# bbuhrow/avx-ecm

Measured on AMD Instinct MI355X. Metric: stage-1 curves/sec at B1=1000000, 416-bit N, higher is better.
Workload: dtype u32 (28-bit limbs, 64-bit accumulate)

## Files before the change

### avx-ecm_amd/csrc/gecm_row.hpp

```cpp
#pragma once
#include "gecm_curve.hpp"
#include "gecm_rowk.h"

template <int NQ>
struct FeR {
    int32_t v[NQ];
};

template <int NQ>
struct RowMod {
    uint32_t n[NQ];
    uint32_t rho;
    int32_t c16;
    int32_t kb, zb;
};

__device__ __forceinline__ void row_pin(const int64_t &x)
{
    asm volatile("" ::"v"(x));
}
__device__ __forceinline__ int32_t row_c16()
{
    int32_t c;
    asm volatile("s_mov_b32 %0, 16" : "=s"(c));
    return c;
}
template <int32_t V>
__device__ __forceinline__ int32_t row_bias()
{
    int32_t c;
    asm volatile("v_mov_b32 %0, %1" : "=v"(c) : "n"(V));
    return c;
}

#define GECM_DPP_ROW_SHL1 0x101
#define GECM_DPP_ROW_SHR1 0x111
#define GECM_DPP_ROW_ROR1 0x121
#define GECM_DPP_ROW_NEWBCAST 0x150

template <int CTRL>
__device__ __forceinline__ uint32_t row_dpp(uint32_t x)
{
    return (uint32_t)__builtin_amdgcn_update_dpp(0, (int)x, CTRL, 0xF, 0xF, true);
}
template <int I>
__device__ __forceinline__ uint32_t row_bcast(uint32_t x)
{
    return row_dpp<GECM_DPP_ROW_NEWBCAST + I>(x);
}
template <int I>
__device__ __forceinline__ int64_t row_bcast64(int64_t x)
{
    return __builtin_amdgcn_update_dpp((int64_t)0, x, GECM_DPP_ROW_NEWBCAST + I, 0xF, 0xF, true);
}
template <int I>
__device__ __forceinline__ uint32_t row_bcast_lds(uint32_t x)
{
    return (uint32_t)__builtin_amdgcn_ds_swizzle((int)x, 0x10 | (I << 5));
}
__device__ __forceinline__ uint32_t other_row(uint32_t x)
{
    return (uint32_t)__builtin_amdgcn_ds_swizzle((int)x, 0x401F );
}

__device__ __forceinline__ void smad(int64_t &acc, int32_t x, int32_t y)
{
    asm("v_mad_i64_i32 %0, vcc, %1, %2, %0" : "+v"(acc) : "v"(x), "v"(y) : "vcc");
}
__device__ __forceinline__ void umad(int64_t &acc, uint32_t x, uint32_t y)
{
    asm("v_mad_u64_u32 %0, vcc, %1, %2, %0" : "+v"(acc) : "v"(x), "v"(y) : "vcc");
}
__device__ __forceinline__ int64_t smad0(int32_t x, int32_t y)
{
    int64_t r;
    asm("v_mad_i64_i32 %0, vcc, %1, %2, 0" : "=v"(r) : "v"(x), "v"(y) : "vcc");
    return r;
}
__device__ __forceinline__ int64_t smad16(int32_t x, int64_t add)
{
    int64_t r;
    asm("v_mad_i64_i32 %0, vcc, %1, 16, %2" : "=v"(r) : "v"(x), "v"(add) : "vcc");
    return r;
}

__device__ __forceinline__ int64_t smad16_smad(int32_t x, int64_t add, int32_t y, int32_t z)
{
    int64_t r;
    asm("v_mad_i64_i32 %0, vcc, %1, 16, %2\n\tv_mad_i64_i32 %0, vcc, %3, %4, %0" : "=&v"(r) : "v"(x), "v"(add), "v"(y), "v"(z) : "vcc");
    return r;
}

template <int ROWS>
struct RowScan {
    int32_t Ab[ROWS];
};

template <int NQ, int ROWS, bool RHO1, bool ALDS, bool A4 = false, bool B4 = false, bool R4 = false, bool SCANNED = false>
__device__ __forceinline__ void fer_mul(FeR<NQ> &r, const FeR<NQ> &a, const FeR<NQ> &b, const RowMod<NQ> &m,
                                        const RowScan<ROWS> *scan = nullptr)
{
    static_assert(ROWS > 16 * (NQ - 1) && ROWS <= 16 * NQ, "the limbs in use fill the lanes but for the last one");
    static_assert(!ALDS || NQ == 1, "the crossbar form is for one limb per lane");
    static_assert(!SCANNED || (NQ == 1 && !ALDS), "a ready-made scan is for the one-limb DPP form");
    int32_t a4[NQ], b4[NQ];
#pragma unroll
    for (int t = 0; t < NQ; t++) {
        a4[t] = A4 ? a.v[t] : (int32_t)((uint32_t)a.v[t] << 2);
        b4[t] = B4 ? b.v[t] : (int32_t)((uint32_t)b.v[t] << 2);
    }
    if constexpr (NQ >= 2) {
        int64_t T[NQ];
        const int64_t a01 = (int64_t)(((uint64_t)(uint32_t)a4[1] << 32) | (uint32_t)a4[0]);
        int64_t Ap = row_bcast64<0>(a01);
        int32_t As = 0;
        auto limb = [&](auto jc) -> int32_t {
            constexpr int q = decltype(jc)::value % NQ;
            return q == 0 ? (int32_t)(uint32_t)Ap : q == 1 ? (int32_t)(Ap >> 32) : As;
        };
#pragma unroll
        for (int t = 0; t < NQ; t++) T[t] = (int64_t)limb(IC<0>{}) * b4[t];
        static_for<0, ROWS>([&](auto ic) {
            constexpr int i = decltype(ic)::value;
            constexpr int rot = i % NQ, nxt = (i + 1) % NQ;
            const uint32_t Q = row_bcast<0>(RHO1 ? (uint32_t)T[rot] : (uint32_t)T[rot] * m.rho);
            __builtin_amdgcn_sched_barrier(0);
#pragma unroll
            for (int t = 0; t < NQ; t++) {
                T[(t + rot) % NQ] = (int64_t)((uint64_t)T[(t + rot) % NQ] + (uint64_t)Q * m.n[t]);
                __builtin_amdgcn_sched_barrier(0);
            }
            const int32_t Ac = limb(IC<i + 1>{});
            if constexpr (i + 1 < ROWS) {
#pragma unroll
                for (int t = 0; t < NQ - 1; t++) {
                    T[(t + nxt) % NQ] += (int64_t)Ac * b4[t];
                    row_pin(T[(t + nxt) % NQ]);
                    __builtin_amdgcn_sched_barrier(0);
                }
            }
            const int32_t hi = (int32_t)(T[rot] >> 32);
            const uint32_t lo = row_dpp<GECM_DPP_ROW_SHL1>((uint32_t)T[rot]);
            __builtin_amdgcn_sched_barrier(0);
            T[nxt] += (int64_t)hi * m.c16;
            row_pin(T[nxt]);
            __builtin_amdgcn_sched_barrier(0);
            if constexpr (i + 1 < ROWS) {
                T[rot] = (int64_t)Ac * b4[NQ - 1] + (int64_t)(uint64_t)lo;
                row_pin(T[rot]);
            } else {
                T[rot] = (int64_t)(uint64_t)lo;
            }
            __builtin_amdgcn_sched_barrier(0);
            if constexpr (i + 2 < ROWS) {
                if constexpr ((i + 2) % NQ == 0) Ap = row_bcast64<(i + 2) / NQ>(a01);
                else if constexpr ((i + 2) % NQ == 2) As = (int32_t)row_bcast<(i + 2) / NQ>((uint32_t)a4[NQ - 1]);
                __builtin_amdgcn_sched_barrier(0);
            }
        });
        int32_t lo[NQ];
        int32_t carry = 0;
#pragma unroll
        for (int t = 0; t < NQ - 1; t++) {
            int64_t u16 = T[(t + ROWS) % NQ] + (int64_t)(1u << 31);
            if (t > 0) u16 += (int64_t)carry * m.c16;
            carry = (int32_t)(u16 >> 32);
            lo[t] = (int32_t)(((uint32_t)u16 >> 4) & GECM_LIMB_MASK) - (1 << 27);
        }
        const int32_t ut = (int32_t)(T[(NQ - 1 + ROWS) % NQ] >> 4) + carry + (1 << 27);
        lo[NQ - 1] = (int32_t)((uint32_t)ut & GECM_LIMB_MASK) - (1 << 27);
        const int32_t below = (int32_t)row_dpp<GECM_DPP_ROW_SHR1>((uint32_t)(ut >> GECM_LIMB_BITS));
        lo[0] += below;
#pragma unroll
        for (int t = 0; t < NQ; t++) r.v[t] = R4 ? (int32_t)((uint32_t)lo[t] << 2) : lo[t];
    } else {
        int32_t Ab[ROWS];
        int64_t a01 = 0;
        if constexpr (SCANNED) {
#pragma unroll
            for (int j = 0; j < ROWS; j++) Ab[j] = scan->Ab[j];
        }
        if constexpr (!ALDS && !SCANNED) a01 = (int64_t)(((uint64_t)row_dpp<GECM_DPP_ROW_SHL1>((uint32_t)a4[0]) << 32) | (uint32_t)a4[0]);
        auto request = [&](auto jc) {
            constexpr int j = decltype(jc)::value;
            if constexpr (SCANNED) {
            } else if constexpr (ALDS) {
                Ab[j] = (int32_t)row_bcast_lds<j>((uint32_t)a4[0]);
            } else if constexpr (j % 2 == 0) {
                const int64_t P = row_bcast64<j>(a01);
                Ab[j] = (int32_t)(uint32_t)P;
                if constexpr (j + 1 < ROWS) Ab[j + 1] = (int32_t)(P >> 32);
            }
        };
        if constexpr (ALDS) static_for<0, ROWS>(request);
        else request(IC<0>{});
        int64_t T[NQ];
#pragma unroll
        for (int t = 0; t < NQ; t++) T[t] = 0;
        static_for<0, ROWS>([&](auto ic) {
            constexpr int i = decltype(ic)::value;
            if constexpr (i == 0) T[0] = smad0(Ab[0], b4[0]);
            if constexpr (!ALDS) {
                __builtin_amdgcn_sched_barrier(0);
                if constexpr (i + 1 < ROWS) request(IC<i + 1>{});
                __builtin_amdgcn_sched_barrier(0);
            }
            uint32_t qs = (uint32_t)T[0];
            if (!RHO1) qs *= m.rho;
            const uint32_t Q = row_bcast<0>(qs);
            umad(T[0], Q, m.n[0]);
            if constexpr (!ALDS) __builtin_amdgcn_sched_barrier(0);
            const int32_t hi = (int32_t)(T[0] >> 32);
            const uint32_t lo = row_dpp<GECM_DPP_ROW_SHL1>((uint32_t)T[0]);
            int64_t add = (int64_t)(uint64_t)lo;
            if constexpr (R4 && i + 2 == ROWS) add = (int64_t)(((uint64_t)(uint32_t)m.kb << 32) | lo);
            if constexpr (R4 && i + 1 == ROWS) add = (int64_t)(((uint64_t)(uint32_t)m.zb << 32) | lo);
            if constexpr (i + 1 < ROWS) T[0] = smad16_smad(hi, add, Ab[i + 1], b4[0]);
            else T[0] = smad16(hi, add);
        });
        if constexpr (R4) {
            r.v[0] = (int32_t)(((uint32_t)T[0] >> 2) + (row_dpp<GECM_DPP_ROW_ROR1>((uint32_t)(T[0] >> 32)) << 2));
        } else {
            const int64_t u16 = T[0] + (int64_t)(1u << 31);
            const int32_t lim = (int32_t)(((uint32_t)u16 >> 4) & GECM_LIMB_MASK) - (1 << 27);
            r.v[0] = lim + (int32_t)row_dpp<GECM_DPP_ROW_SHR1>((uint32_t)(u16 >> 32));
        }
    }
}

template <int ROWS>
__device__ __forceinline__ void fer_scan(RowScan<ROWS> &s, const FeR<1> &a)
{
    const int64_t a01 = (int64_t)(((uint64_t)row_dpp<GECM_DPP_ROW_SHL1>((uint32_t)a.v[0]) << 32) | (uint32_t)a.v[0]);
    static_for<0, (ROWS + 1) / 2>([&](auto kc) {
        constexpr int j = 2 * decltype(kc)::value;
        const int64_t P = row_bcast64<j>(a01);
        s.Ab[j] = (int32_t)(uint32_t)P;
        if constexpr (j + 1 < ROWS) s.Ab[j + 1] = (int32_t)(P >> 32);
    });
    __builtin_amdgcn_sched_barrier(0);
}
template <int ROWS>
__device__ __forceinline__ void fer_mul_scanned(FeR<1> &r, const RowScan<ROWS> &s, const FeR<1> &b, const RowMod<1> &m)
{
    fer_mul<1, ROWS, true, false, true, true, true, true>(r, b, b, m, &s);
}

template <int NQ>
struct PtR {
    FeR<NQ> own;
    FeR<NQ> oth;
};

struct RowSign {
    uint32_t mz, bz;
    uint32_t mx, bx;
};

template <int NQ>
__device__ __forceinline__ void fer_other(FeR<NQ> &r, const FeR<NQ> &a)
{
#pragma unroll
    for (int t = 0; t < NQ; t++) r.v[t] = (int32_t)other_row((uint32_t)a.v[t]);
}

template <int NQ>
__device__ __forceinline__ void fer_sum_diff(FeR<NQ> &r, const FeR<NQ> &oth, const FeR<NQ> &own, const RowSign &g)
{
#pragma unroll
    for (int t = 0; t < NQ; t++) r.v[t] = (int32_t)((uint32_t)oth.v[t] + ((uint32_t)own.v[t] ^ g.mz) + g.bz);
}

template <int NQ>
__device__ __forceinline__ void row_sd(FeR<NQ> &r, const PtR<NQ> &p, const RowSign &g)
{
    fer_sum_diff<NQ>(r, p.oth, p.own, g);
}

template <int NQ>
__device__ __forceinline__ void row_ds(FeR<NQ> &r, const PtR<NQ> &p, const RowSign &g)
{
#pragma unroll
    for (int t = 0; t < NQ; t++) r.v[t] = (int32_t)((uint32_t)p.own.v[t] + ((uint32_t)p.oth.v[t] ^ g.mx) + g.bx);
}

template <int NQ>
__device__ __forceinline__ void row_pick(FeR<NQ> &r, const FeR<NQ> &a, const FeR<NQ> &b, uint64_t pick)
{
#pragma unroll
    for (int t = 0; t < NQ; t++) {
        int32_t x;
        asm volatile("v_cndmask_b32 %0, %1, %2, %3" : "=v"(x) : "v"(a.v[t]), "v"(b.v[t]), "s"(pick));
        r.v[t] = x;
    }
}

template <int NQ, int ROWS, bool ALDS>
__device__ __forceinline__ void row_add(FeR<NQ> &own, const FeR<NQ> &fB, const FeR<NQ> &fA, const FeR<NQ> &c, bool isZ,
                                        const RowSign &g, const RowMod<NQ> &m)
{
    FeR<NQ> w, t, e;
    fer_mul<NQ, ROWS, true, ALDS, true, true, true>(w, fB, fA, m);
    fer_other<NQ>(t, w);
    fer_sum_diff<NQ>(e, t, w, g);
    fer_mul<NQ, ROWS, true, ALDS, true, true, true>(e, e, e, m);
    fer_mul<NQ, ROWS, true, ALDS, true, true, true>(own, e, c, m);
}

template <int ROWS, class Shadow>
__device__ __forceinline__ void row_add_scanned(FeR<1> &own, const RowScan<ROWS> &sA, const FeR<1> &fB, const FeR<1> &c,
                                                const RowSign &g, const RowMod<1> &m, Shadow &&shadow)
{
    FeR<1> w, t, e;
    RowScan<ROWS> sC;
    fer_mul_scanned<ROWS>(w, sA, fB, m);
    fer_other<1>(t, w);
    fer_scan<ROWS>(sC, c);
    shadow();
    __builtin_amdgcn_sched_barrier(0);
    fer_sum_diff<1>(e, t, w, g);
    fer_mul<1, ROWS, true, false, true, true, true>(e, e, e, m);
    fer_mul_scanned<ROWS>(own, sC, e, m);
}

template <int NQ, int ROWS, bool ALDS>
__device__ __forceinline__ void row_dup(FeR<NQ> &own, const FeR<NQ> &fA, const FeR<NQ> &s4, bool isZ, const RowSign &g,
                                        const RowMod<NQ> &m)
{
    FeR<NQ> q, t, w, p1, p2, r1;
    fer_mul<NQ, ROWS, true, ALDS, true, true, true>(q, fA, fA, m);
    fer_other<NQ>(t, q);
#pragma unroll
    for (int i = 0; i < NQ; i++) {
        w.v[i] = t.v[i] - q.v[i];
        p1.v[i] = isZ ? s4.v[i] : q.v[i];
        p2.v[i] = isZ ? w.v[i] : t.v[i];
    }
    fer_mul<NQ, ROWS, true, ALDS, true, true, true>(r1, p1, p2, m);
#pragma unroll
    for (int i = 0; i < NQ; i++) t.v[i] = r1.v[i] + q.v[i];
    fer_mul<NQ, ROWS, true, ALDS, true, true, true>(t, t, w, m);
#pragma unroll
    for (int i = 0; i < NQ; i++) own.v[i] = isZ ? t.v[i] : r1.v[i];
}

template <int NQ>
__device__ __forceinline__ void fer_load(FeR<NQ> &r, const uint32_t *__restrict__ base, size_t stride, uint32_t cidx,
                                         uint32_t l, uint32_t nl)
{
#pragma unroll
    for (int t = 0; t < NQ; t++) {
        const uint32_t limb = (uint32_t)NQ * l + (uint32_t)t;
        r.v[t] = limb < nl ? (int32_t)base[(size_t)limb * stride + cidx] : 0;
    }
}

template <int NQ, int ROWS, bool ALDS>
__device__ __forceinline__ void run_tape_row(const uint32_t *__restrict__ tape, uint32_t tape_len, PtR<NQ> &A,
                                             const FeR<NQ> &s4, bool isZ, const RowSign &g, const RowMod<NQ> &m)
{
    PtR<NQ> B = A;
    FeR<NQ> Coth = A.oth;
    auto fetch = [&](uint32_t pc) -> uint32_t {
        uint32_t w = tape[pc >> 2];
        return __builtin_amdgcn_readfirstlane((w >> ((pc & 3u) * 8u)) & 0xffu);
    };
    uint32_t nxt = tape_len ? fetch(0) : GECM_OP_NOP;
    for (uint32_t pc = 0; pc < tape_len; pc++) {
        uint32_t op = nxt;
        nxt = (pc + 1 < tape_len) ? fetch(pc + 1) : GECM_OP_NOP;
        while ((op & ~GECM_OP_SWAP) == (GECM_OP_STEP | GECM_OP_RULE3)) {
            const uint64_t swap = (op & GECM_OP_SWAP) ? ~(uint64_t)0 : 0;
            FeR<NQ> fA, fB;
            if constexpr (NQ == 1 && !ALDS) {
                RowScan<ROWS> sA;
                row_sd<NQ>(fA, A, g);
                row_pick<NQ>(A.own, A.own, B.own, swap);
                fer_scan<ROWS>(sA, fA);
                row_ds<NQ>(fB, B, g);
                row_add_scanned<ROWS>(B.own, sA, fB, Coth, g, m, [&]() {
                    row_pick<NQ>(Coth, B.oth, A.oth, swap);
                    row_pick<NQ>(A.oth, A.oth, B.oth, swap);
                });
                pc++;
                op = nxt;
                nxt = (pc + 1 < tape_len) ? fetch(pc + 1) : GECM_OP_NOP;
                __builtin_amdgcn_sched_barrier(0);
                fer_other<NQ>(B.oth, B.own);
            } else {
                row_sd<NQ>(fA, A, g);
                row_ds<NQ>(fB, B, g);
                row_pick<NQ>(A.own, A.own, B.own, swap);
                row_add<NQ, ROWS, ALDS>(B.own, fB, fA, Coth, isZ, g, m);
                row_pick<NQ>(Coth, B.oth, A.oth, swap);
                row_pick<NQ>(A.oth, A.oth, B.oth, swap);
                fer_other<NQ>(B.oth, B.own);
                pc++;
                op = nxt;
                nxt = (pc + 1 < tape_len) ? fetch(pc + 1) : GECM_OP_NOP;
            }
        }
        if (op == GECM_OP_NOP) continue;
        const uint32_t rule = op & GECM_OP_RULE_MASK;
        const bool is_step = op >= GECM_OP_STEP;
        const bool do_add = op != GECM_OP_PRAC_BEGIN;
        const bool do_dup = op != GECM_OP_PRAC_END;
        PtR<NQ> C;
        C.oth = Coth;
        fer_other<NQ>(C.own, Coth);
        if (is_step && (op & GECM_OP_SWAP)) {
            PtR<NQ> t = A;
            A = B;
            B = t;
        }
        if (is_step && rule == GECM_OP_RULE5) {
            PtR<NQ> t = B;
            B = C;
            C = t;
        } else if (is_step && rule == GECM_OP_RULE9) {
            PtR<NQ> t = A;
            A = B;
            B = C;
            C = t;
        } else if (op == GECM_OP_PRAC_BEGIN) {
            B = A;
            C = A;
        }
        PtR<NQ> T, D;
        FeR<NQ> fA, fB;
        row_sd<NQ>(fA, A, g);
        row_ds<NQ>(fB, B, g);
        if (do_add) {
            if constexpr (NQ == 1 && !ALDS) {
                RowScan<ROWS> sA;
                fer_scan<ROWS>(sA, fA);
                row_add_scanned<ROWS>(T.own, sA, fB, C.oth, g, m, []() {});
            } else {
                row_add<NQ, ROWS, ALDS>(T.own, fB, fA, C.oth, isZ, g, m);
            }
            fer_other<NQ>(T.oth, T.own);
        }
        if (do_dup) {
            row_dup<NQ, ROWS, ALDS>(D.own, fA, s4, isZ, g, m);
            fer_other<NQ>(D.oth, D.own);
        }
        if (op == GECM_OP_PRAC_END) {
            A = T;
        } else if (op == GECM_OP_PRAC_BEGIN) {
            A = D;
        } else if (rule == GECM_OP_RULE4) {
            B = T;
            A = D;
        } else if (rule == GECM_OP_RULE5) {
            PtR<NQ> t = C;
            C = T;
            B = t;
            A = D;
        } else {
            PtR<NQ> oldA = C;
            C = T;
            B = D;
            A = oldA;
        }
        Coth = C.oth;
    }
}


template <int NQ, int ROWS, bool ALDS>
__device__ __forceinline__ void stage1_row(const uint32_t *__restrict__ tape, uint32_t tape_len, uint32_t *__restrict__ X,
                                           uint32_t *__restrict__ Z, const uint32_t *__restrict__ S, size_t stride,
                                           uint32_t nl, const uint32_t *__restrict__ rc, uint32_t rho_n)
{
    const uint32_t cidx = (blockIdx.x * blockDim.x + threadIdx.x) >> 5;
    const uint32_t l = threadIdx.x & 15u;
    const bool isZ = (threadIdx.x & 16u) != 0;
    uint32_t *mine = isZ ? Z : X;
    RowMod<NQ> mp, mn;
    FeR<NQ> cin, one, kp;
#pragma unroll
    for (int t = 0; t < NQ; t++) {
        const uint32_t j = (uint32_t)NQ * l + (uint32_t)t;
        mp.n[t] = rc[0 * GECM_ROW_WORDS + j];
        mn.n[t] = rc[1 * GECM_ROW_WORDS + j];
        cin.v[t] = (int32_t)rc[2 * GECM_ROW_WORDS + j];
        one.v[t] = (int32_t)rc[3 * GECM_ROW_WORDS + j];
        kp.v[t] = (int32_t)rc[4 * GECM_ROW_WORDS + j];
    }
    mp.rho = 1u;
    mn.rho = rho_n;
    mp.c16 = mn.c16 = row_c16();
    mp.kb = mn.kb = mp.zb = mn.zb = 0;
    if constexpr (NQ == 1) {
        mp.kb = mn.kb = row_bias<(1 << 27)>();
        mp.zb = mn.zb = row_bias<-(1 << 27)>();
    }
    PtR<NQ> P;
    FeR<NQ> s4, t;
    fer_load<NQ>(t, mine, stride, cidx, l, nl);
    fer_mul<NQ, ROWS, true, ALDS, false, false, true>(P.own, t, cin, mp);
    RowSign g;
    g.mz = isZ ? 0xffffffffu : 0u;
    g.bz = isZ ? 1u : 0u;
    g.mx = ~g.mz;
    g.bx = 1u - g.bz;
    fer_other<NQ>(P.oth, P.own);
    fer_load<NQ>(t, S, stride, cidx, l, nl);
    fer_mul<NQ, ROWS, true, ALDS, false, false, true>(s4, t, cin, mp);
    run_tape_row<NQ, ROWS, ALDS>(tape, tape_len, P, s4, isZ, g, mp);
    fer_mul<NQ, ROWS, false, ALDS, true>(t, P.own, one, mn);
    uint32_t u[NQ];
#pragma unroll
    for (int i = 0; i < NQ; i++) u[i] = (uint32_t)(t.v[i] + kp.v[i]);
    const uint32_t below = row_dpp<GECM_DPP_ROW_SHR1>(u[NQ - 1] >> GECM_LIMB_BITS);
#pragma unroll
    for (int i = 0; i < NQ; i++) {
        const uint32_t limb = (uint32_t)NQ * l + (uint32_t)i;
        const uint32_t v = (u[i] & GECM_LIMB_MASK) + (i == 0 ? below : (u[i - 1] >> GECM_LIMB_BITS));
        if (limb < nl) mine[(size_t)limb * stride + cidx] = (limb == nl - 1) ? v + (u[i] & ~GECM_LIMB_MASK) : v;
    }
}


template <int NQ, int ROWS>
__device__ __forceinline__ void fer_reduce(FeR<NQ> &v, const RowMod<NQ> &m, float minv, uint32_t l)
{
    constexpr int TL = (ROWS - 1) / NQ, TS = (ROWS - 1) % NQ;
    const int32_t top = (int32_t)row_bcast<TL>((uint32_t)v.v[TS]);
    const int32_t q = (int32_t)__builtin_rintf((float)top * minv);
    int32_t lo[NQ], c[NQ];
#pragma unroll
    for (int t = 0; t < NQ; t++) {
        const int32_t x = v.v[t] - q * (int32_t)m.n[t];
        const bool split = (uint32_t)NQ * l + (uint32_t)t < (uint32_t)(ROWS - 1);
        c[t] = split ? (x + (1 << 27)) >> GECM_LIMB_BITS : 0;
        lo[t] = x - (int32_t)((uint32_t)c[t] << GECM_LIMB_BITS);
    }
    v.v[0] = lo[0] + (int32_t)row_dpp<GECM_DPP_ROW_SHR1>((uint32_t)c[NQ - 1]);
#pragma unroll
    for (int t = 1; t < NQ; t++) v.v[t] = lo[t] + c[t - 1];
}

template <int NQ>
struct UnitRow {
    RowMod<NQ> m;
    FeR<NQ> two;
    float minv;
    uint32_t l;
    bool pp1;
};

template <int NQ, int ROWS>
__device__ __forceinline__ void unit_row_add(FeR<NQ> &T, const FeR<NQ> &X, const FeR<NQ> &Y, const FeR<NQ> &W,
                                             const UnitRow<NQ> &u)
{
    fer_mul<NQ, ROWS, true, false>(T, X, Y, u.m);
    if (u.pp1) {
#pragma unroll
        for (int t = 0; t < NQ; t++) T.v[t] -= W.v[t];
        fer_reduce<NQ, ROWS>(T, u.m, u.minv, u.l);
    }
}

template <int NQ, int ROWS>
__device__ __forceinline__ void run_tape_unit_row(const uint32_t *__restrict__ tape, uint32_t tape_len, FeR<NQ> &A,
                                                  const UnitRow<NQ> &u)
{
    FeR<NQ> B = A, C = A;
    auto fetch = [&](uint32_t pc) -> uint32_t {
        uint32_t w = tape[pc >> 2];
        return __builtin_amdgcn_readfirstlane((w >> ((pc & 3u) * 8u)) & 0xffu);
    };
    uint32_t nxt = tape_len ? fetch(0) : GECM_OP_NOP;
    for (uint32_t pc = 0; pc < tape_len; pc++) {
        uint32_t op = nxt;
        nxt = (pc + 1 < tape_len) ? fetch(pc + 1) : GECM_OP_NOP;
        while ((op & ~GECM_OP_SWAP) == (GECM_OP_STEP | GECM_OP_RULE3)) {
            if (op & GECM_OP_SWAP) {
                FeR<NQ> t = A;
                A = B;
                B = t;
            }
            FeR<NQ> T;
            unit_row_add<NQ, ROWS>(T, B, A, C, u);
            C = B;
            B = T;
            pc++;
            op = nxt;
            nxt = (pc + 1 < tape_len) ? fetch(pc + 1) : GECM_OP_NOP;
        }
        if (op == GECM_OP_NOP) continue;
        const uint32_t rule = op & GECM_OP_RULE_MASK;
        const bool is_step = op >= GECM_OP_STEP;
        const bool do_add = op != GECM_OP_PRAC_BEGIN;
        const bool do_dup = op != GECM_OP_PRAC_END;
        if (is_step && (op & GECM_OP_SWAP)) {
            FeR<NQ> t = A;
            A = B;
            B = t;
        }
        if (is_step && rule == GECM_OP_RULE5) {
            FeR<NQ> t = B;
            B = C;
            C = t;
        } else if (is_step && rule == GECM_OP_RULE9) {
            FeR<NQ> t = A;
            A = B;
            B = C;
            C = t;
        } else if (op == GECM_OP_PRAC_BEGIN) {
            B = A;
            C = A;
        }
        FeR<NQ> T, D;
        if (do_add) unit_row_add<NQ, ROWS>(T, B, A, C, u);
        if (do_dup) unit_row_add<NQ, ROWS>(D, A, A, u.two, u);
        if (op == GECM_OP_PRAC_END) {
            A = T;
        } else if (op == GECM_OP_PRAC_BEGIN) {
            A = D;
        } else if (rule == GECM_OP_RULE4) {
            B = T;
            A = D;
        } else if (rule == GECM_OP_RULE5) {
            FeR<NQ> t = C;
            C = T;
            B = t;
            A = D;
        } else {
            FeR<NQ> oldA = C;
            C = T;
            B = D;
            A = oldA;
        }
    }
}

template <int NQ, int ROWS>
__device__ __forceinline__ void unit_row(const uint32_t *__restrict__ tape, uint32_t tape_len, uint32_t *__restrict__ X,
                                         size_t stride, uint32_t nl, bool pp1, const uint32_t *__restrict__ rc)
{
    const uint32_t pos = (blockIdx.x * blockDim.x + threadIdx.x) >> 4;
    const uint32_t l = threadIdx.x & 15u;
    UnitRow<NQ> u;
    RowMod<NQ> mn;
    FeR<NQ> cin, one, kp;
#pragma unroll
    for (int t = 0; t < NQ; t++) {
        const uint32_t j = (uint32_t)NQ * l + (uint32_t)t;
        u.m.n[t] = rc[0 * GECM_ROW_WORDS + j];
        mn.n[t] = rc[1 * GECM_ROW_WORDS + j];
        cin.v[t] = (int32_t)rc[2 * GECM_ROW_WORDS + j];
        one.v[t] = (int32_t)rc[3 * GECM_ROW_WORDS + j];
        kp.v[t] = (int32_t)rc[4 * GECM_ROW_WORDS + j];
        u.two.v[t] = (int32_t)rc[5 * GECM_ROW_WORDS + j];
    }
    u.minv = __uint_as_float(rc[6 * GECM_ROW_WORDS + 0]);
    u.m.rho = 1u;
    mn.rho = rc[6 * GECM_ROW_WORDS + 1];
    u.m.c16 = mn.c16 = row_c16();
    u.l = l;
    u.pp1 = pp1;
    FeR<NQ> A, t;
    fer_load<NQ>(t, X, stride, pos, l, nl);
    fer_mul<NQ, ROWS, true, false>(A, t, cin, u.m);
    fer_reduce<NQ, ROWS>(A, u.m, u.minv, l);
    run_tape_unit_row<NQ, ROWS>(tape, tape_len, A, u);
    fer_mul<NQ, ROWS, false, false>(t, A, one, mn);
    uint32_t w[NQ];
#pragma unroll
    for (int i = 0; i < NQ; i++) w[i] = (uint32_t)(t.v[i] + kp.v[i]);
    const uint32_t below = row_dpp<GECM_DPP_ROW_SHR1>(w[NQ - 1] >> GECM_LIMB_BITS);
#pragma unroll
    for (int i = 0; i < NQ; i++) {
        const uint32_t limb = (uint32_t)NQ * l + (uint32_t)i;
        const uint32_t v = (w[i] & GECM_LIMB_MASK) + (i == 0 ? below : (w[i - 1] >> GECM_LIMB_BITS));
        if (limb < nl) X[(size_t)limb * stride + pos] = (limb == nl - 1) ? v + (w[i] & ~GECM_LIMB_MASK) : v;
    }
}
```

Before: 1716.

## Add specialized DPP tape interpreter reusing scanned operand across add and dup

Adds a dedicated tape interpreter for the single-limb-per-lane, non-LDS row path. It shares the prefix scan of fA between the differential add and the doubling, and adds a scanned variant of the doubling routine. The rule 4/5/9 point permutations become branchless lane selects driven by bitmasks instead of struct swaps. This is meant to cut redundant scans and data movement per PRAC step, at the cost of more select instructions and a larger special-case code path to keep correct.

Result: faster. 1747, median of 6 (+1.8%).

```diff
diff --git a/avx-ecm_amd/csrc/gecm_row.hpp b/avx-ecm_amd/csrc/gecm_row.hpp
--- a/avx-ecm_amd/csrc/gecm_row.hpp
+++ b/avx-ecm_amd/csrc/gecm_row.hpp
@@ -344,6 +344,25 @@
     for (int i = 0; i < NQ; i++) own.v[i] = isZ ? t.v[i] : r1.v[i];
 }
 
+template <int ROWS>
+__device__ __forceinline__ void row_dup_scanned(FeR<1> &own, const RowScan<ROWS> &sA, const FeR<1> &fA, const FeR<1> &s4,
+                                                bool isZ, const RowMod<1> &m)
+{
+    FeR<1> q, t, w, p1, p2, r1;
+    RowScan<ROWS> sP, sW;
+    fer_mul_scanned<ROWS>(q, sA, fA, m);
+    fer_other<1>(t, q);
+    p1.v[0] = isZ ? s4.v[0] : q.v[0];
+    fer_scan<ROWS>(sP, p1);
+    w.v[0] = t.v[0] - q.v[0];
+    p2.v[0] = isZ ? w.v[0] : t.v[0];
+    fer_mul_scanned<ROWS>(r1, sP, p2, m);
+    t.v[0] = r1.v[0] + q.v[0];
+    fer_scan<ROWS>(sW, w);
+    fer_mul_scanned<ROWS>(t, sW, t, m);
+    own.v[0] = isZ ? t.v[0] : r1.v[0];
+}
+
 template <int NQ>
 __device__ __forceinline__ void fer_load(FeR<NQ> &r, const uint32_t *__restrict__ base, size_t stride, uint32_t cidx,
                                          uint32_t l, uint32_t nl)
@@ -355,10 +374,107 @@
     }
 }
 
+template <int ROWS>
+__device__ __forceinline__ void run_tape_row_dpp(const uint32_t *__restrict__ tape, uint32_t tape_len, PtR<1> &A,
+                                                 const FeR<1> &s4, bool isZ, const RowSign &g, const RowMod<1> &m)
+{
+    PtR<1> B = A;
+    FeR<1> Coth = A.oth;
+    auto fetch = [&](uint32_t pc) -> uint32_t {
+        uint32_t w = tape[pc >> 2];
+        return __builtin_amdgcn_readfirstlane((w >> ((pc & 3u) * 8u)) & 0xffu);
+    };
+    uint32_t pc = 0;
+    uint32_t op = tape_len ? fetch(0) : GECM_OP_NOP;
+    uint32_t nxt = 1 < tape_len ? fetch(1) : GECM_OP_NOP;
+    auto advance = [&]() {
+        pc++;
+        op = nxt;
+        nxt = (pc + 1 < tape_len) ? fetch(pc + 1) : GECM_OP_NOP;
+        __builtin_amdgcn_sched_barrier(0);
+    };
+    while (pc < tape_len) {
+        while ((op & ~GECM_OP_SWAP) == (GECM_OP_STEP | GECM_OP_RULE3)) {
+            const uint64_t swap = (op & GECM_OP_SWAP) ? ~(uint64_t)0 : 0;
+            FeR<1> fA, fB;
+            RowScan<ROWS> sA;
+            row_sd<1>(fA, A, g);
+            row_pick<1>(A.own, A.own, B.own, swap);
+            fer_scan<ROWS>(sA, fA);
+            row_ds<1>(fB, B, g);
+            row_add_scanned<ROWS>(B.own, sA, fB, Coth, g, m, [&]() {
+                row_pick<1>(Coth, B.oth, A.oth, swap);
+                row_pick<1>(A.oth, A.oth, B.oth, swap);
+            });
+            advance();
+            fer_other<1>(B.oth, B.own);
+        }
+        if (op == GECM_OP_NOP) {
+            advance();
+            continue;
+        }
+        FeR<1> fA, fB;
+        RowScan<ROWS> sA;
+        if (op == GECM_OP_PRAC_END) {
+            row_sd<1>(fA, A, g);
+            fer_scan<ROWS>(sA, fA);
+            row_ds<1>(fB, B, g);
+            row_add_scanned<ROWS>(A.own, sA, fB, Coth, g, m, []() {});
+            advance();
+            fer_other<1>(A.oth, A.own);
+            continue;
+        }
+        if (op == GECM_OP_PRAC_BEGIN) {
+            row_sd<1>(fA, A, g);
+            fer_scan<ROWS>(sA, fA);
+            B = A;
+            Coth = A.oth;
+            row_dup_scanned<ROWS>(A.own, sA, fA, s4, isZ, m);
+            advance();
+            fer_other<1>(A.oth, A.own);
+            continue;
+        }
+        const bool r59 = (op & GECM_OP_RULE_MASK) != GECM_OP_RULE4, r9 = (op & GECM_OP_RULE_MASK) == GECM_OP_RULE9;
+        const uint64_t swap = (uint64_t)0 - (((op >> 2) ^ ((op >> 1) & op)) & 1u);
+        const uint64_t rot = (uint64_t)0 - ((op >> 1) & 1u);
+        PtR<1> a, b, q;
+        FeR<1> Cown, c, T, Toth;
+        asm volatile("" : "=v"(Cown.v[0]));
+        if (r59) fer_other<1>(Cown, Coth);
+        row_pick<1>(a.own, A.own, B.own, swap);
+        row_pick<1>(a.oth, A.oth, B.oth, swap);
+        row_sd<1>(fA, a, g);
+        fer_scan<ROWS>(sA, fA);
+        row_pick<1>(b.own, B.own, A.own, swap);
+        row_pick<1>(b.oth, B.oth, A.oth, swap);
+        row_pick<1>(q.own, b.own, Cown, rot);
+        row_pick<1>(q.oth, b.oth, Coth, rot);
+        row_pick<1>(c, Coth, b.oth, rot);
+        row_ds<1>(fB, q, g);
+        row_add_scanned<ROWS>(T, sA, fB, c, g, m, []() {});
+        fer_other<1>(Toth, T);
+        row_dup_scanned<ROWS>(A.own, sA, fA, s4, isZ, m);
+        advance();
+        fer_other<1>(A.oth, A.own);
+        row_pick<1>(B.own, T, b.own, rot);
+        row_pick<1>(B.oth, Toth, b.oth, rot);
+        row_pick<1>(Coth, Coth, Toth, rot);
+        if (r9) {
+            const PtR<1> t = A;
+            A = B;
+            B = t;
+        }
+    }
+}
+
 template <int NQ, int ROWS, bool ALDS>
 __device__ __forceinline__ void run_tape_row(const uint32_t *__restrict__ tape, uint32_t tape_len, PtR<NQ> &A,
                                              const FeR<NQ> &s4, bool isZ, const RowSign &g, const RowMod<NQ> &m)
 {
+    if constexpr (NQ == 1 && !ALDS) {
+        run_tape_row_dpp<ROWS>(tape, tape_len, A, s4, isZ, g, m);
+        return;
+    }
     PtR<NQ> B = A;
     FeR<NQ> Coth = A.oth;
     auto fetch = [&](uint32_t pc) -> uint32_t {
@@ -372,33 +488,16 @@
         while ((op & ~GECM_OP_SWAP) == (GECM_OP_STEP | GECM_OP_RULE3)) {
             const uint64_t swap = (op & GECM_OP_SWAP) ? ~(uint64_t)0 : 0;
             FeR<NQ> fA, fB;
-            if constexpr (NQ == 1 && !ALDS) {
-                RowScan<ROWS> sA;
-                row_sd<NQ>(fA, A, g);
-                row_pick<NQ>(A.own, A.own, B.own, swap);
-                fer_scan<ROWS>(sA, fA);
-                row_ds<NQ>(fB, B, g);
-                row_add_scanned<ROWS>(B.own, sA, fB, Coth, g, m, [&]() {
-                    row_pick<NQ>(Coth, B.oth, A.oth, swap);
-                    row_pick<NQ>(A.oth, A.oth, B.oth, swap);
-                });
-                pc++;
-                op = nxt;
-                nxt = (pc + 1 < tape_len) ? fetch(pc + 1) : GECM_OP_NOP;
-                __builtin_amdgcn_sched_barrier(0);
-                fer_other<NQ>(B.oth, B.own);
-            } else {
-                row_sd<NQ>(fA, A, g);
-                row_ds<NQ>(fB, B, g);
-                row_pick<NQ>(A.own, A.own, B.own, swap);
-                row_add<NQ, ROWS, ALDS>(B.own, fB, fA, Coth, isZ, g, m);
-                row_pick<NQ>(Coth, B.oth, A.oth, swap);
-                row_pick<NQ>(A.oth, A.oth, B.oth, swap);
-                fer_other<NQ>(B.oth, B.own);
-                pc++;
-                op = nxt;
-                nxt = (pc + 1 < tape_len) ? fetch(pc + 1) : GECM_OP_NOP;
-            }
+            row_sd<NQ>(fA, A, g);
+            row_ds<NQ>(fB, B, g);
+            row_pick<NQ>(A.own, A.own, B.own, swap);
+            row_add<NQ, ROWS, ALDS>(B.own, fB, fA, Coth, isZ, g, m);
+            row_pick<NQ>(Coth, B.oth, A.oth, swap);
+            row_pick<NQ>(A.oth, A.oth, B.oth, swap);
+            fer_other<NQ>(B.oth, B.own);
+            pc++;
+            op = nxt;
+            nxt = (pc + 1 < tape_len) ? fetch(pc + 1) : GECM_OP_NOP;
         }
         if (op == GECM_OP_NOP) continue;
         const uint32_t rule = op & GECM_OP_RULE_MASK;
@@ -431,13 +530,7 @@
         row_sd<NQ>(fA, A, g);
         row_ds<NQ>(fB, B, g);
         if (do_add) {
-            if constexpr (NQ == 1 && !ALDS) {
-                RowScan<ROWS> sA;
-                fer_scan<ROWS>(sA, fA);
-                row_add_scanned<ROWS>(T.own, sA, fB, C.oth, g, m, []() {});
-            } else {
-                row_add<NQ, ROWS, ALDS>(T.own, fB, fA, C.oth, isZ, g, m);
-            }
+            row_add<NQ, ROWS, ALDS>(T.own, fB, fA, C.oth, isZ, g, m);
             fer_other<NQ>(T.oth, T.own);
         }
         if (do_dup) {
```
